# V-DETR/V-DETR

Hardware: AMD Instinct MI355X
Metric: scenes/sec (train fwd+bwd) 40k-pt ScanNet (higher is better)
Workload: dtype f32

## Files before the change

### v-detr_amd/csrc/attn_fwd_pipe.hip

```cpp
#include "attn_common.h"

namespace vdetr {

constexpr int kPT = 10;
constexpr int kPCells = kPT * kPT * kPT;
constexpr int kPipeThreads = 512;
constexpr int kPipeWaves = kPipeThreads / kWave;
constexpr int kPipePad = 20;
constexpr int kLdsPad = kRpeVerts * kPCells * 16;
constexpr int kLdsMl = kLdsPad + kPipeWaves * 16 * kPipePad * 4;
constexpr int kLdsXch = kLdsMl + kPipeWaves * 4 * 8 * 4;
constexpr int kLdsNext = kLdsXch + kPipeWaves * 8 * kWave * 4;
constexpr int kPipeLdsBytes = kLdsNext + 16;
constexpr int kPipeZeroCell = kPipeLdsBytes / 16;
constexpr int kPipeLdsBytesNearest = kPipeLdsBytes + 16;
static_assert(kPipeLdsBytes % 16 == 0 && kPipeLdsBytesNearest <= 160 * 1024, "the zero cell is a 16-byte slot inside the 160 KB LDS");

typedef float f32x2 __attribute__((ext_vector_type(2)));

struct PipeArgs {
  AttnParams P;
  unsigned* counter;
  int nitems, qtiles;
  const char* kv_img;
  int q_f32;
};

__device__ __forceinline__ AxisTap pipe_axis(float d, float log_scale, float pix_mul, float pix_add) {
  const float L = __log2f(__builtin_fmaf(fabsf(d), log_scale, 1.0f));
  const float pix = __builtin_fmaf(copysignf(L, d), pix_mul, pix_add);
  const float bf = __builtin_amdgcn_fmed3f(floorf(pix), 0.f, (float)(kPT - 2));
  const float t = pix - bf;
  AxisTap a;
  a.base = (int)bf;
  a.wa = sat01(1.f - fabsf(t));
  a.wb = sat01(1.f - fabsf(t - 1.f));
  return a;
}

struct PipeCorners {
  f32x4 c[8];
};
__device__ __forceinline__ void pipe_read8(const f32x4* t, PipeCorners& C) {
  C.c[0] = t[0]; C.c[1] = t[1]; C.c[2] = t[kPT]; C.c[3] = t[kPT + 1];
  C.c[4] = t[kPT * kPT]; C.c[5] = t[kPT * kPT + 1]; C.c[6] = t[kPT * kPT + kPT]; C.c[7] = t[kPT * kPT + kPT + 1];
}
__device__ __forceinline__ void pipe_fma8(const PipeCorners& C, float axa, float axb, float w00, float w01, float w10, float w11,
                                          f32x2& s01, f32x2& s23) {
  const float w[8] = {axa * w00, axb * w00, axa * w01, axb * w01, axa * w10, axb * w10, axa * w11, axb * w11};
#pragma unroll
  for (int k = 0; k < 8; ++k) {
    s01 = __builtin_elementwise_fma(f32x2{C.c[k][0], C.c[k][1]}, f32x2{w[k], w[k]}, s01);
    s23 = __builtin_elementwise_fma(f32x2{C.c[k][2], C.c[k][3]}, f32x2{w[k], w[k]}, s23);
  }
}

struct PipeQuery {
  float x0, x1, y0, y1, z0, z1;
  float rc, rs;
};

template <bool ROT, bool NEAREST>
__device__ __forceinline__ void pipe_bias_box(const AttnParams& P, const f32x4* tab, const PipeQuery& Q, float kx, float ky, float kz,
                                              f32x2& s01, f32x2& s23) {
  float dx[2], dy[2], dz[2];
  if (ROT) {
    float ax0 = Q.x0 - kx, ay0 = Q.y0 - ky;
    rpe_rotate(ax0, ay0, Q.rc, Q.rs);
    dx[0] = ax0; dx[1] = ax0 + Q.x1;
    dy[0] = ay0; dy[1] = ay0 + Q.y1;
    dz[0] = Q.z0 - kz; dz[1] = dz[0] + Q.z1;
  } else {
    dx[0] = Q.x0 - kx; dx[1] = Q.x1 - kx;
    dy[0] = Q.y0 - ky; dy[1] = Q.y1 - ky;
    dz[0] = Q.z0 - kz; dz[1] = Q.z1 - kz;
  }
  if constexpr (NEAREST) {
    int cx[2], cy[2], cz[2];
#pragma unroll
    for (int a = 0; a < 2; ++a) {
      cx[a] = rpe_axis_nearest(dx[a], P.log_scale, P.pix_mul, P.pix_add, kPT, 1);
      cy[a] = rpe_axis_nearest(dy[a], P.log_scale, P.pix_mul, P.pix_add, kPT, kPT);
      cz[a] = rpe_axis_nearest(dz[a], P.log_scale, P.pix_mul, P.pix_add, kPT, kPT * kPT);
    }
    f32x4 cv[kRpeVerts];
#pragma unroll
    for (int i = 0; i < kRpeVerts; ++i)
      cv[i] = tab[min(i * kPCells + cz[rpe_box_zi(i)] + cy[rpe_box_yi(i)] + cx[rpe_box_xi(i)], kPipeZeroCell)];
#pragma unroll
    for (int i = 0; i < kRpeVerts; ++i) {
      s01 += f32x2{cv[i][0], cv[i][1]};
      s23 += f32x2{cv[i][2], cv[i][3]};
    }
    return;
  }
  const AxisTap ax[2] = {pipe_axis(dx[0], P.log_scale, P.pix_mul, P.pix_add), pipe_axis(dx[1], P.log_scale, P.pix_mul, P.pix_add)};
  const AxisTap ay[2] = {pipe_axis(dy[0], P.log_scale, P.pix_mul, P.pix_add), pipe_axis(dy[1], P.log_scale, P.pix_mul, P.pix_add)};
  const AxisTap az[2] = {pipe_axis(dz[0], P.log_scale, P.pix_mul, P.pix_add), pipe_axis(dz[1], P.log_scale, P.pix_mul, P.pix_add)};
  float w00[2][2], w01[2][2], w10[2][2], w11[2][2];
  int zy[2][2];
#pragma unroll
  for (int zi = 0; zi < 2; ++zi)
#pragma unroll
    for (int yi = 0; yi < 2; ++yi) {
      w00[zi][yi] = az[zi].wa * ay[yi].wa; w01[zi][yi] = az[zi].wa * ay[yi].wb;
      w10[zi][yi] = az[zi].wb * ay[yi].wa; w11[zi][yi] = az[zi].wb * ay[yi].wb;
      zy[zi][yi] = __mul24(__mul24(az[zi].base, kPT) + ay[yi].base, kPT);
    }
  PipeCorners cur, nxt;
  pipe_read8(tab + zy[rpe_box_zi(0)][rpe_box_yi(0)] + ax[rpe_box_xi(0)].base, cur);
#pragma unroll
  for (int i = 0; i < kRpeVerts; ++i) {
    const int xi = rpe_box_xi(i), yi = rpe_box_yi(i), zi = rpe_box_zi(i);
    if (i + 1 < kRpeVerts)
      pipe_read8(tab + (i + 1) * kPCells + zy[rpe_box_zi(i + 1)][rpe_box_yi(i + 1)] + ax[rpe_box_xi(i + 1)].base, nxt);
    __builtin_amdgcn_sched_barrier(0);
    pipe_fma8(cur, ax[xi].wa, ax[xi].wb, w00[zi][yi], w01[zi][yi], w10[zi][yi], w11[zi][yi], s01, s23);
    if (i + 1 < kRpeVerts) cur = nxt;
  }
}

template <bool NEAREST>
__device__ __forceinline__ void pipe_bias_general(const AttnParams& P, const f32x4* tab, const float* __restrict__ vp, bool rot, float rc,
                                                  float rs, float kx, float ky, float kz, f32x2& s01, f32x2& s23) {
#pragma unroll 1
  for (int i = 0; i < kRpeVerts; ++i) {
    float dx = vp[i * 3] - kx, dy = vp[i * 3 + 1] - ky;
    const float dz = vp[i * 3 + 2] - kz;
    if (rot) rpe_rotate(dx, dy, rc, rs);
    if constexpr (NEAREST) {
      const int cell = rpe_axis_nearest(dx, P.log_scale, P.pix_mul, P.pix_add, kPT, 1) +
                       rpe_axis_nearest(dy, P.log_scale, P.pix_mul, P.pix_add, kPT, kPT) +
                       rpe_axis_nearest(dz, P.log_scale, P.pix_mul, P.pix_add, kPT, kPT * kPT);
      const f32x4 cv = tab[min(i * kPCells + cell, kPipeZeroCell)];
      s01 += f32x2{cv[0], cv[1]};
      s23 += f32x2{cv[2], cv[3]};
      continue;
    }
    const AxisTap ax = pipe_axis(dx, P.log_scale, P.pix_mul, P.pix_add), ay = pipe_axis(dy, P.log_scale, P.pix_mul, P.pix_add),
                  az = pipe_axis(dz, P.log_scale, P.pix_mul, P.pix_add);
    PipeCorners C;
    pipe_read8(tab + i * kPCells + (az.base * kPT + ay.base) * kPT + ax.base, C);
    pipe_fma8(C, ax.wa, ax.wb, az.wa * ay.wa, az.wa * ay.wb, az.wb * ay.wa, az.wb * ay.wb, s01, s23);
  }
}

__device__ __forceinline__ float pipe_give_back(float v, bool swapped, bool odd_row) {
  const auto r = __builtin_amdgcn_permlane16_swap(__float_as_uint(v), __float_as_uint(v), false, false);
  const float other = __uint_as_float(odd_row ? r[0] : r[1]);
  return swapped ? other : v;
}

enum { kPipeBox = 0, kPipeBoxRot = 1, kPipeGeneral = 2 };

typedef __bf16 bf16x8 __attribute__((ext_vector_type(8)));
typedef __bf16 bf16x4 __attribute__((ext_vector_type(4)));
typedef short short4v __attribute__((ext_vector_type(4)));

constexpr int pipe_k_pieces(int split) { return split == 1 ? 2 : 6; }
constexpr int pipe_v_pieces(int split) { return split == 1 ? 2 : 4; }
constexpr int pipe_tile_bytes(int split) { return (pipe_k_pieces(split) + pipe_v_pieces(split)) * kWave * 16; }

template <int SPLIT>
struct PipeTileT {
  f32x4 kb[SPLIT ? 1 : 4], vb[SPLIT ? 1 : 4];
  bf16x8 k8[SPLIT ? pipe_k_pieces(SPLIT) : 1];
  f32x4 v8[SPLIT ? pipe_v_pieces(SPLIT) : 1];
  float kx, ky, kz;
};

__device__ __forceinline__ void split3(float x, __bf16& h, __bf16& m, __bf16& l) {
  h = (__bf16)x;
  const float r1 = x - (float)h;
  m = (__bf16)r1;
  l = (__bf16)(r1 - (float)m);
}

struct PipeLane {
  const float* kp;
  const float* vp;
  const float* xp;
  float* sp;
  const char* img;
};

template <int SPLIT>
__device__ __forceinline__ void pipe_fetch_k(const AttnParams& P, const PipeLane& A, int tile, int nK, int c, PipeTileT<SPLIT>& t) {
  if constexpr (SPLIT) {
    const char* src = A.img + (size_t)tile * pipe_tile_bytes(SPLIT);
#pragma unroll
    for (int j = 0; j < pipe_k_pieces(SPLIT); ++j) t.k8[j] = *reinterpret_cast<const bf16x8*>(src + j * kWave * 16);
  } else {
    const int kc = min((tile << 4) + c, nK - 1) - c;
    const f32x4* kp = reinterpret_cast<const f32x4*>(A.kp + kc * P.k_stride);
#pragma unroll
    for (int s4 = 0; s4 < 4; ++s4) t.kb[s4] = kp[s4];
  }
}
template <int SPLIT>
__device__ __forceinline__ void pipe_fetch_x(const PipeLane& A, int tile, int nK, int c, PipeTileT<SPLIT>& t) {
  const int kc = min((tile << 4) + c, nK - 1) - c;
  const float* xp = A.xp + kc * 3;
  t.kx = xp[0]; t.ky = xp[1]; t.kz = xp[2];
}
template <int SPLIT>
__device__ __forceinline__ void pipe_fetch_v(const AttnParams& P, const PipeLane& A, int tile, int nK, int g, PipeTileT<SPLIT>& t) {
  if constexpr (SPLIT) {
    const char* src = A.img + (size_t)tile * pipe_tile_bytes(SPLIT) + pipe_k_pieces(SPLIT) * kWave * 16;
#pragma unroll
    for (int j = 0; j < pipe_v_pieces(SPLIT); ++j) t.v8[j] = *reinterpret_cast<const f32x4*>(src + j * kWave * 16);
  } else {
#pragma unroll
    for (int s = 0; s < 4; ++s) {
      const int kk = min((tile << 4) + 4 * g + s, nK - 1) - 4 * g;
      t.vb[s] = *reinterpret_cast<const f32x4*>(A.vp + kk * P.v_stride);
    }
  }
}

template <int SPLIT>
struct PipeQT {
  float qa[SPLIT ? 1 : 16];
  bf16x8 q8[SPLIT ? pipe_k_pieces(SPLIT) : 1];
};

template <int MODE, bool TAIL, int SPLIT, bool NEAREST>
__device__ __forceinline__ void pipe_tile(const AttnParams& P, const f32x4* tab, float* ppad, const PipeLane& A, const PipeQuery& Q,
                                          const float* __restrict__ role_vp, const PipeQT<SPLIT>& QA, PipeTileT<SPLIT>& ops, int tile, int next, int b,
                                          int qrow, int g, int c, bool swapped, f32x4 (&o)[4], float (&m)[4], float (&l)[4]) {
  const int nK = P.nK;
  const int key = (tile << 4) + c;
  const bool kvalid = !TAIL || key < nK;
  f32x4 acc = {0.f, 0.f, 0.f, 0.f};
  if constexpr (SPLIT == 1) {
    acc = __builtin_amdgcn_mfma_f32_16x16x32_bf16(QA.q8[0], ops.k8[0], acc, 0, 0, 0);
    acc = __builtin_amdgcn_mfma_f32_16x16x32_bf16(QA.q8[1], ops.k8[1], acc, 0, 0, 0);
    acc *= P.scale;
  } else if constexpr (SPLIT) {
    constexpr int kTerms[6][2] = {{2, 0}, {0, 2}, {1, 1}, {1, 0}, {0, 1}, {0, 0}};
#pragma unroll
    for (int t = 0; t < 6; ++t)
#pragma unroll
      for (int mm = 0; mm < 2; ++mm)
        acc = __builtin_amdgcn_mfma_f32_16x16x32_bf16(QA.q8[2 * kTerms[t][0] + mm], ops.k8[2 * kTerms[t][1] + mm], acc, 0, 0, 0);
  } else {
#pragma unroll
    for (int s = 0; s < 16; ++s) acc = __builtin_amdgcn_mfma_f32_16x16x4f32(QA.qa[s], ops.kb[s >> 2][s & 3], acc, 0, 0, 0);
  }
  if constexpr (!SPLIT) pipe_fetch_k<SPLIT>(P, A, next, nK, c, ops);
  const float kx = ops.kx, ky = ops.ky, kz = ops.kz;
  pipe_fetch_x<SPLIT>(A, next, nK, c, ops);
  f32x2 s01 = {0.f, 0.f}, s23 = {0.f, 0.f};
  if (MODE == kPipeGeneral) pipe_bias_general<NEAREST>(P, tab, role_vp, P.cos_sin != nullptr, Q.rc, Q.rs, kx, ky, kz, s01, s23);
  else pipe_bias_box<MODE == kPipeBoxRot, NEAREST>(P, tab, Q, kx, ky, kz, s01, s23);
  if constexpr (SPLIT) {
    __builtin_amdgcn_sched_barrier(0);
    pipe_fetch_k<SPLIT>(P, A, next, nK, c, ops);
    __builtin_amdgcn_sched_barrier(0);
  }
  const bool odd = g & 1;
  float sc[4];
  sc[0] = acc[0] + pipe_give_back(s01[0], swapped, odd);
  sc[1] = acc[1] + pipe_give_back(s01[1], swapped, odd);
  sc[2] = acc[2] + pipe_give_back(s23[0], swapped, odd);
  sc[3] = acc[3] + pipe_give_back(s23[1], swapped, odd);
  if (TAIL && !kvalid) {
#pragma unroll
    for (int r = 0; r < 4; ++r) sc[r] = kNegBig;
  }
  if (A.sp && kvalid && qrow < P.nQ) {
    float* sp = A.sp + (tile << 4);
#pragma unroll
    for (int r = 0; r < 4; ++r) {
      __builtin_nontemporal_store(sc[r], sp + r * nK);
    }
  }
  float p[4];
#pragma unroll
  for (int r = 0; r < 4; ++r) {
    const float tmax = row_allmax_f32_fx(sc[r]);
    const float mn = fmaxf(m[r], tmax);
    const float alpha = __expf(m[r] - mn);
    const float e = kvalid ? __expf(sc[r] - mn) : 0.f;
    l[r] = l[r] * alpha + row_allsum_f32_fx(e);
    m[r] = mn;
    p[r] = e;
#pragma unroll
    for (int t = 0; t < 4; ++t) o[t][r] *= alpha;
  }
  if (P.drop_thresh) {
    const uint4 rnd = attn_rand4(P, b, qrow, key, 0);
    p[0] = rnd.x >= P.drop_thresh ? p[0] * P.drop_scale : 0.f;
    p[1] = rnd.y >= P.drop_thresh ? p[1] * P.drop_scale : 0.f;
    p[2] = rnd.z >= P.drop_thresh ? p[2] * P.drop_scale : 0.f;
    p[3] = rnd.w >= P.drop_thresh ? p[3] * P.drop_scale : 0.f;
  }
#pragma unroll
  for (int r = 0; r < 4; ++r) ppad[(4 * g + r) * kPipePad + c] = p[r];
  __builtin_amdgcn_wave_barrier();
  const f32x4 pa = *reinterpret_cast<const f32x4*>(ppad + c * kPipePad + 4 * g);
  __builtin_amdgcn_wave_barrier();
  if constexpr (SPLIT == 1) {
    const bf16x4 pb = {(__bf16)pa[0], (__bf16)pa[1], (__bf16)pa[2], (__bf16)pa[3]};
    const short4v ab = __builtin_bit_cast(short4v, pb);
    typedef short short8v __attribute__((ext_vector_type(8)));
#pragma unroll
    for (int t = 0; t < 4; ++t) {
      const short8v vv = __builtin_bit_cast(short8v, ops.v8[t >> 1]);
      const short4v vt = (t & 1) ? short4v{vv[4], vv[5], vv[6], vv[7]} : short4v{vv[0], vv[1], vv[2], vv[3]};
      o[t] = __builtin_amdgcn_mfma_f32_16x16x16bf16_1k(ab, vt, o[t], 0, 0, 0);
    }
  } else if constexpr (SPLIT) {
    bf16x4 ph, pl;
#pragma unroll
    for (int e = 0; e < 4; ++e) {
      const __bf16 h = (__bf16)pa[e];
      ph[e] = h;
      pl[e] = (__bf16)(pa[e] - (float)h);
    }
    const short4v ah = __builtin_bit_cast(short4v, ph), al = __builtin_bit_cast(short4v, pl);
#pragma unroll
    for (int t = 0; t < 4; ++t) {
      typedef short short8v __attribute__((ext_vector_type(8)));
      const short8v vv = __builtin_bit_cast(short8v, ops.v8[t]);
      const short4v vh = {vv[0], vv[1], vv[2], vv[3]}, vl = {vv[4], vv[5], vv[6], vv[7]};
      o[t] = __builtin_amdgcn_mfma_f32_16x16x16bf16_1k(al, vh, o[t], 0, 0, 0);
      o[t] = __builtin_amdgcn_mfma_f32_16x16x16bf16_1k(ah, vl, o[t], 0, 0, 0);
      o[t] = __builtin_amdgcn_mfma_f32_16x16x16bf16_1k(ah, vh, o[t], 0, 0, 0);
    }
  } else {
#pragma unroll
    for (int t = 0; t < 4; ++t)
#pragma unroll
      for (int s = 0; s < 4; ++s) o[t] = __builtin_amdgcn_mfma_f32_16x16x4f32(pa[s], ops.vb[s][t], o[t], 0, 0, 0);
  }
  pipe_fetch_v<SPLIT>(P, A, next, nK, g, ops);
}

template <int MODE, int SPLIT, bool NEAREST>
__device__ __forceinline__ void pipe_tiles(const AttnParams& P, const f32x4* tab, float* ppad, const PipeLane& A, const PipeQuery& Q,
                                           const float* __restrict__ role_vp, const PipeQT<SPLIT>& qa, PipeTileT<SPLIT>& ops, int tile_begin,
                                           int tile_end, int w, int b, int qrow, int g, int c, bool swapped, f32x4 (&o)[4],
                                           float (&m)[4], float (&l)[4]) {
  const int nK = P.nK;
  const int full_end = min(tile_end, nK >> 4);
  int tile = tile_begin + w;
  for (; tile < full_end; tile += kPipeWaves) {
    const int next = tile + kPipeWaves < tile_end ? tile + kPipeWaves : tile;
    pipe_tile<MODE, false, SPLIT, NEAREST>(P, tab, ppad, A, Q, role_vp, qa, ops, tile, next, b, qrow, g, c, swapped, o, m, l);
  }
  if (tile < tile_end)
    pipe_tile<MODE, true, SPLIT, NEAREST>(P, tab, ppad, A, Q, role_vp, qa, ops, tile, tile, b, qrow, g, c, swapped, o, m, l);
}

template <bool ROT, int SPLIT, bool NEAREST = false>
__global__ __launch_bounds__(kPipeThreads) void attn_fwd_rpe_pipe_kernel(PipeArgs K) {
  extern __shared__ __attribute__((aligned(16))) float smem[];
  AttnParams& P = K.P;
  attn_load_rng(P);
  const int tid = threadIdx.x, lane = tid & 63;
  const int w = __builtin_amdgcn_readfirstlane(tid >> 6);
  const int g = lane >> 4, c = lane & 15;
  const bool swapped = c >= 4 && c < 12;
  const int gq = swapped ? (g ^ 1) : g;
  const int nQ = P.nQ, nK = P.nK, H = 4;
  const f32x4* tab = reinterpret_cast<const f32x4*>(smem);
  float* ppad = smem + kLdsPad / 4 + w * (16 * kPipePad);
  float* mlbuf = smem + kLdsMl / 4;
  float* xch = smem + kLdsXch / 4;
  volatile int* nextbuf = reinterpret_cast<volatile int*>(smem + kLdsNext / 4);

  const int last_draw = K.nitems + (int)gridDim.x - 1;
  if (tid == 0) {
    const int first = (int)atomicAdd(K.counter, 1u);
    nextbuf[0] = first;
    if (first == last_draw) atomicExch(K.counter, 0u);
  }
  if ((int)blockIdx.x + 8 >= (int)gridDim.x) {
    __syncthreads();
    if (nextbuf[0] >= K.nitems) return;
  }
  rpe_stage_table(P, reinterpret_cast<f32x4*>(smem), tid, kPipeThreads);
  if (NEAREST && tid == 0) reinterpret_cast<f32x4*>(smem)[kPipeZeroCell] = f32x4{0.f, 0.f, 0.f, 0.f};
  __syncthreads();
  int item = nextbuf[0];
  int parity = 0;
  const int ntiles = (nK + 15) >> 4;
  const int qstride = H * kDh;

  while (item < K.nitems) {
    int drawn = 0;
    if (tid == 0) drawn = (int)atomicAdd(K.counter, 1u);
    const int split = item % P.ksplit;
    const int qt = (item / P.ksplit) % K.qtiles;
    const int b = item / (P.ksplit * K.qtiles);
    const int q0 = qt * 4;
    const int tile_begin = split * P.tiles_per_split;
    const int tile_end = min(ntiles, tile_begin + P.tiles_per_split);
    const int qrow = q0 + g;
    const int q_role = min(q0 + gq, nQ - 1);
    PipeQT<SPLIT> qa;
    {
      const int qi = min(q0 + (c >> 2), nQ - 1);
      const float* qrowp = P.q + ((size_t)b * nQ + qi) * qstride + (c & 3) * kDh;
      if constexpr (SPLIT == 1) {
        if (K.q_f32) {
#pragma unroll
          for (int mm = 0; mm < 2; ++mm) {
            const f32x4* src = reinterpret_cast<const f32x4*>(qrowp + 32 * mm + 8 * g);
            const f32x4 v0 = src[0], v1 = src[1];
#pragma unroll
            for (int e = 0; e < 8; ++e) qa.q8[mm][e] = (__bf16)(e < 4 ? v0[e] : v1[e - 4]);
          }
        } else {
          const __bf16* qb = reinterpret_cast<const __bf16*>(P.q) + ((size_t)b * nQ + qi) * qstride + (c & 3) * kDh;
          qa.q8[0] = *reinterpret_cast<const bf16x8*>(qb + 8 * g);
          qa.q8[1] = *reinterpret_cast<const bf16x8*>(qb + 32 + 8 * g);
        }
      } else if constexpr (SPLIT) {
#pragma unroll
        for (int mm = 0; mm < 2; ++mm) {
          const f32x4* src = reinterpret_cast<const f32x4*>(qrowp + 32 * mm + 8 * g);
          const f32x4 v0 = src[0], v1 = src[1];
#pragma unroll
          for (int e = 0; e < 8; ++e) {
            __bf16 h, md, lo;
            split3((e < 4 ? v0[e] : v1[e - 4]) * P.scale, h, md, lo);
            qa.q8[mm][e] = h; qa.q8[2 + mm][e] = md; qa.q8[4 + mm][e] = lo;
          }
        }
      } else {
        const f32x4* src = reinterpret_cast<const f32x4*>(qrowp + 16 * g);
#pragma unroll
        for (int s4 = 0; s4 < 4; ++s4) {
          const f32x4 v = src[s4];
#pragma unroll
          for (int e = 0; e < 4; ++e) qa.qa[s4 * 4 + e] = v[e] * P.scale;
        }
      }
    }
    const float* role_vp = P.vertices + ((size_t)b * nQ + q_role) * 24;
    PipeQuery Q;
    Q.rc = 1.f; Q.rs = 0.f;
    bool box;
    {
      float vx[8], vy[8], vz[8];
#pragma unroll
      for (int i = 0; i < 8; ++i) { vx[i] = role_vp[i * 3]; vy[i] = role_vp[i * 3 + 1]; vz[i] = role_vp[i * 3 + 2]; }
      if (ROT) {
        Q.rc = P.cos_sin[((size_t)b * nQ + q_role) * 2];
        Q.rs = P.cos_sin[((size_t)b * nQ + q_role) * 2 + 1];
        float ex, ey, ez;
        box = __all(rpe_box_pattern_rot(vx, vy, vz, Q.rc, Q.rs, ex, ey, ez));
        Q.x0 = vx[0]; Q.y0 = vy[0]; Q.z0 = vz[0];
        Q.x1 = ex; Q.y1 = ey; Q.z1 = ez;
      } else {
        box = __all(rpe_box_pattern(vx, vy, vz));
        Q.x0 = vx[0]; Q.x1 = vx[2]; Q.y0 = vy[0]; Q.y1 = vy[1]; Q.z0 = vz[0]; Q.z1 = vz[4];
      }
    }
    PipeLane A;
    A.kp = P.k + ((size_t)b * nK + c) * P.k_stride + 16 * g;
    A.vp = P.v + ((size_t)b * nK + 4 * g) * P.v_stride + 4 * c;
    A.xp = P.xyz + ((size_t)b * nK + c) * 3;
    A.sp = P.scores ? P.scores + (((size_t)b * nQ + min(qrow, nQ - 1)) * H) * nK + c : nullptr;
    A.img = SPLIT ? K.kv_img + ((size_t)b * ntiles) * pipe_tile_bytes(SPLIT) + lane * 16 : nullptr;

    f32x4 o[4];
#pragma unroll
    for (int t = 0; t < 4; ++t) o[t] = f32x4{0.f, 0.f, 0.f, 0.f};
    float m[4] = {kNegBig, kNegBig, kNegBig, kNegBig}, l[4] = {0.f, 0.f, 0.f, 0.f};
    PipeTileT<SPLIT> ops;
    {
      const int t0 = min(tile_begin + w, ntiles - 1);
      pipe_fetch_k<SPLIT>(P, A, t0, nK, c, ops);
      pipe_fetch_x<SPLIT>(A, t0, nK, c, ops);
      pipe_fetch_v<SPLIT>(P, A, t0, nK, g, ops);
    }
    if (box)
      pipe_tiles<ROT ? kPipeBoxRot : kPipeBox, SPLIT, NEAREST>(P, tab, ppad, A, Q, role_vp, qa, ops, tile_begin, tile_end, w, b, qrow, g, c, swapped, o, m, l);
    else
      pipe_tiles<kPipeGeneral, SPLIT, NEAREST>(P, tab, ppad, A, Q, role_vp, qa, ops, tile_begin, tile_end, w, b, qrow, g, c, swapped, o, m, l);

    if (tid == 0) {
      nextbuf[parity ^ 1] = drawn;
      if (drawn == last_draw) atomicExch(K.counter, 0u);
    }
    __syncthreads();
    if (c == 0) {
      float* mine = mlbuf + (w * 4 + g) * 8;
      *reinterpret_cast<f32x4*>(mine) = f32x4{m[0], m[1], m[2], m[3]};
      *reinterpret_cast<f32x4*>(mine + 4) = f32x4{l[0], l[1], l[2], l[3]};
    }
    const int own_t = w >> 1, own_hi = w & 1;
#pragma unroll
    for (int half = 0; half < 2; ++half) {
      if (half) __syncthreads();
#pragma unroll
      for (int t = 0; t < 4; ++t)
#pragma unroll
        for (int hi = 0; hi < 2; ++hi) xch[(w * 8 + t * 2 + hi) * kWave + lane] = o[t][2 * hi + half];
      __syncthreads();
      const int r = 2 * own_hi + half;
      float M = kNegBig;
      float mw[kPipeWaves], lw[kPipeWaves];
#pragma unroll
      for (int ww = 0; ww < kPipeWaves; ++ww) {
        mw[ww] = mlbuf[(ww * 4 + g) * 8 + r];
        lw[ww] = mlbuf[(ww * 4 + g) * 8 + 4 + r];
        M = fmaxf(M, mw[ww]);
      }
      float L = 0.f, val = 0.f;
#pragma unroll
      for (int ww = 0; ww < kPipeWaves; ++ww) {
        const float f = __expf(mw[ww] - M);
        L += lw[ww] * f;
        val += xch[(ww * 8 + own_t * 2 + own_hi) * kWave + lane] * f;
      }
      if (qrow < nQ) {
        const float inv = L > 0.f ? 1.f / L : 0.f;
        const float lse = L > 0.f ? M + __logf(L) : kNegBig;
        const int d = 4 * c + own_t;
        const size_t row = ((size_t)b * nQ + qrow) * H + r;
        if (P.ksplit == 1) {
          P.out[row * kDh + d] = val * inv;
          if (own_t == 0 && c == 0) P.lse[row] = lse;
        } else {
          const size_t rows = (size_t)P.B * nQ * H;
          P.part_o[((size_t)split * rows + row) * kDh + d] = val * inv;
          if (own_t == 0 && c == 0) P.part_lse[(size_t)split * rows + row] = lse;
        }
      }
    }
    parity ^= 1;
    item = nextbuf[parity];
  }
}


template <int SPLIT, bool SRC_F32 = (SPLIT != 1)>
__global__ __launch_bounds__(kWave) void attn_fwd_pack_kv_kernel(const void* __restrict__ kin, const void* __restrict__ vin, int nK, int k_stride,
                                                                 int v_stride, char* __restrict__ img, long layer_stride, int nB) {
  const int lane = threadIdx.x, g = lane >> 4, c = lane & 15;
  const int tile = blockIdx.x, b = blockIdx.y, ntiles = gridDim.x;
  {
    const size_t esz = SRC_F32 ? 4 : 2;
    kin = reinterpret_cast<const char*>(kin) + (size_t)blockIdx.z * layer_stride * esz;
    vin = reinterpret_cast<const char*>(vin) + (size_t)blockIdx.z * layer_stride * esz;
    img += (size_t)blockIdx.z * nB * ntiles * pipe_tile_bytes(SPLIT);
  }
  char* dst = img + ((size_t)b * ntiles + tile) * pipe_tile_bytes(SPLIT) + lane * 16;
  const int key = tile * 16 + c;
  constexpr int kK = pipe_k_pieces(SPLIT);
  if constexpr (SPLIT == 1 && SRC_F32) {
    const float* k = reinterpret_cast<const float*>(kin);
    const float* v = reinterpret_cast<const float*>(vin);
    const float* kr = k + ((size_t)b * nK + min(key, nK - 1)) * k_stride;
#pragma unroll
    for (int mm = 0; mm < 2; ++mm) {
      const f32x4 v0 = *reinterpret_cast<const f32x4*>(kr + 32 * mm + 8 * g), v1 = *reinterpret_cast<const f32x4*>(kr + 32 * mm + 8 * g + 4);
      bf16x8 h;
#pragma unroll
      for (int e = 0; e < 8; ++e) h[e] = (__bf16)(key < nK ? (e < 4 ? v0[e] : v1[e - 4]) : 0.f);
      *reinterpret_cast<bf16x8*>(dst + mm * kWave * 16) = h;
    }
#pragma unroll
    for (int tp = 0; tp < 2; ++tp) {
      bf16x8 both;
#pragma unroll
      for (int e = 0; e < 4; ++e) {
        const int kk = tile * 16 + 4 * g + e;
        const float* vr = v + ((size_t)b * nK + min(kk, nK - 1)) * v_stride + 4 * c + 2 * tp;
        both[e] = (__bf16)(kk < nK ? vr[0] : 0.f);
        both[4 + e] = (__bf16)(kk < nK ? vr[1] : 0.f);
      }
      *reinterpret_cast<bf16x8*>(dst + (kK + tp) * kWave * 16) = both;
    }
  } else if constexpr (SPLIT == 1) {
    const __bf16* k = reinterpret_cast<const __bf16*>(kin);
    const __bf16* v = reinterpret_cast<const __bf16*>(vin);
    const __bf16* kr = k + ((size_t)b * nK + min(key, nK - 1)) * k_stride;
    const bf16x8 zero8 = {0, 0, 0, 0, 0, 0, 0, 0};
#pragma unroll
    for (int mm = 0; mm < 2; ++mm)
      *reinterpret_cast<bf16x8*>(dst + mm * kWave * 16) = key < nK ? *reinterpret_cast<const bf16x8*>(kr + 32 * mm + 8 * g) : zero8;
#pragma unroll
    for (int tp = 0; tp < 2; ++tp) {
      bf16x8 both;
#pragma unroll
      for (int e = 0; e < 4; ++e) {
        const int kk = tile * 16 + 4 * g + e;
        const __bf16* vr = v + ((size_t)b * nK + min(kk, nK - 1)) * v_stride + 4 * c + 2 * tp;
        both[e] = kk < nK ? vr[0] : (__bf16)0.f;
        both[4 + e] = kk < nK ? vr[1] : (__bf16)0.f;
      }
      *reinterpret_cast<bf16x8*>(dst + (kK + tp) * kWave * 16) = both;
    }
  } else {
    const float* k = reinterpret_cast<const float*>(kin);
    const float* v = reinterpret_cast<const float*>(vin);
    const float* kr = k + ((size_t)b * nK + min(key, nK - 1)) * k_stride;
#pragma unroll
    for (int mm = 0; mm < 2; ++mm) {
      const f32x4 v0 = *reinterpret_cast<const f32x4*>(kr + 32 * mm + 8 * g), v1 = *reinterpret_cast<const f32x4*>(kr + 32 * mm + 8 * g + 4);
      bf16x8 h, md, lo;
#pragma unroll
      for (int e = 0; e < 8; ++e) {
        __bf16 a0, a1, a2;
        split3(key < nK ? (e < 4 ? v0[e] : v1[e - 4]) : 0.f, a0, a1, a2);
        h[e] = a0; md[e] = a1; lo[e] = a2;
      }
      *reinterpret_cast<bf16x8*>(dst + (0 + mm) * kWave * 16) = h;
      *reinterpret_cast<bf16x8*>(dst + (2 + mm) * kWave * 16) = md;
      *reinterpret_cast<bf16x8*>(dst + (4 + mm) * kWave * 16) = lo;
    }
#pragma unroll
    for (int t = 0; t < 4; ++t) {
      bf16x4 h, lo;
#pragma unroll
      for (int e = 0; e < 4; ++e) {
        const int kk = tile * 16 + 4 * g + e;
        const float x = kk < nK ? v[((size_t)b * nK + kk) * v_stride + 4 * c + t] : 0.f;
        const __bf16 hh = (__bf16)x;
        h[e] = hh;
        lo[e] = (__bf16)(x - (float)hh);
      }
      bf16x8 both = {h[0], h[1], h[2], h[3], lo[0], lo[1], lo[2], lo[3]};
      *reinterpret_cast<bf16x8*>(dst + (kK + t) * kWave * 16) = both;
    }
  }
}

}

using namespace vdetr;

namespace vdetr {
size_t attn_fwd_pipe_img_bytes(int B, int nK, int split) { return (size_t)B * ((nK + 15) / 16) * (split == 1 ? pipe_tile_bytes(1) : pipe_tile_bytes(3)); }

int attn_fwd_pack_launch(const void* k, const void* v, int B, int nK, int k_stride, int v_stride, int nlayers, long layer_stride, char* img,
                         int split, bool src_f32, hipStream_t st) {
  const dim3 pg((nK + 15) / 16, B, nlayers);
  if (split == 1 && src_f32) hipLaunchKernelGGL((attn_fwd_pack_kv_kernel<1, true>), pg, dim3(kWave), 0, st, k, v, nK, k_stride, v_stride, img, layer_stride, B);
  else if (split == 1) hipLaunchKernelGGL((attn_fwd_pack_kv_kernel<1, false>), pg, dim3(kWave), 0, st, k, v, nK, k_stride, v_stride, img, layer_stride, B);
  else hipLaunchKernelGGL(attn_fwd_pack_kv_kernel<3>, pg, dim3(kWave), 0, st, k, v, nK, k_stride, v_stride, img, layer_stride, B);
  return check_launch("attn_fwd_pack_kv");
}

int attn_fwd_pipe_launch(const AttnParams& P, unsigned* counter, int workgroups, char* kv_img, int split, bool packed, bool src_f32, hipStream_t st) {
  PipeArgs K;
  K.P = P;
  K.counter = counter;
  K.qtiles = (P.nQ + 3) / 4;
  K.nitems = P.B * K.qtiles * P.ksplit;
  K.kv_img = kv_img;
  K.q_f32 = src_f32 ? 1 : 0;
  const int grid = workgroups < K.nitems ? workgroups : K.nitems;
  if (split && !packed) {
    if (int e = attn_fwd_pack_launch(P.k, P.v, P.B, P.nK, P.k_stride, P.v_stride, 1, 0, kv_img, split, src_f32, st)) return e;
  }
#define VDETR_PIPE_LAUNCH(ROT, SPLIT)                                                                                       \
  do {                                                                                                                      \
    if (P.rpe_nearest) {                                                                                                    \
      if (int e = set_lds(attn_fwd_rpe_pipe_kernel<ROT, SPLIT, true>, kPipeLdsBytesNearest, "attn_fwd")) return e;         \
      hipLaunchKernelGGL((attn_fwd_rpe_pipe_kernel<ROT, SPLIT, true>), dim3(grid), dim3(kPipeThreads), kPipeLdsBytesNearest, st, K); \
    } else {                                                                                                                \
      if (int e = set_lds(attn_fwd_rpe_pipe_kernel<ROT, SPLIT>, kPipeLdsBytes, "attn_fwd")) return e;                      \
      hipLaunchKernelGGL((attn_fwd_rpe_pipe_kernel<ROT, SPLIT>), dim3(grid), dim3(kPipeThreads), kPipeLdsBytes, st, K);    \
    }                                                                                                                       \
  } while (0)
  if (P.cos_sin) {
    if (split == 1) VDETR_PIPE_LAUNCH(true, 1); else if (split) VDETR_PIPE_LAUNCH(true, 3); else VDETR_PIPE_LAUNCH(true, 0);
  } else {
    if (split == 1) VDETR_PIPE_LAUNCH(false, 1); else if (split) VDETR_PIPE_LAUNCH(false, 3); else VDETR_PIPE_LAUNCH(false, 0);
  }
#undef VDETR_PIPE_LAUNCH
  return check_launch("attn_fwd_pipe");
}
}
```

Before: 156.6.

## Prefetch next work item's K/V, query rows and vertices across persistent-loop boundary

The persistent attention forward kernel now draws two work items up front. It prefetches the next item's first K/V/xyz tile inside the last tile iteration and stages that item's query rows, box vertices and cos/sin into LDS during the epilogue, which hides the refill latency between items. The RPE table load is issued into registers before the first synchronisation, item decoding uses precomputed magic-number division, and an optional compile-time timeline instrumentation is added. This adds about 4.5 KB of LDS and extra register pressure, and it makes the counter handling more intricate.

```diff
diff --git a/v-detr_amd/csrc/attn_fwd_pipe.hip b/v-detr_amd/csrc/attn_fwd_pipe.hip
--- a/v-detr_amd/csrc/attn_fwd_pipe.hip
+++ b/v-detr_amd/csrc/attn_fwd_pipe.hip
@@ -11,10 +11,15 @@
 constexpr int kLdsMl = kLdsPad + kPipeWaves * 16 * kPipePad * 4;
 constexpr int kLdsXch = kLdsMl + kPipeWaves * 4 * 8 * 4;
 constexpr int kLdsNext = kLdsXch + kPipeWaves * 8 * kWave * 4;
-constexpr int kPipeLdsBytes = kLdsNext + 16;
+constexpr int kLdsStage = kLdsNext + 16;
+constexpr int kPipeStageFloats = 4 * 256 + 4 * 24 + 4 * 2;
+constexpr int kPipeLdsBytes = kLdsStage + kPipeStageFloats * 4;
 constexpr int kPipeZeroCell = kPipeLdsBytes / 16;
 constexpr int kPipeLdsBytesNearest = kPipeLdsBytes + 16;
 static_assert(kPipeLdsBytes % 16 == 0 && kPipeLdsBytesNearest <= 160 * 1024, "the zero cell is a 16-byte slot inside the 160 KB LDS");
+static_assert(kLdsPad == kRpeVerts * kPCells * 16 && kLdsMl - kLdsPad == kPipeWaves * 16 * kPipePad * 4 && kLdsXch - kLdsMl == 1024 &&
+                  kLdsNext - kLdsXch == 16384 && kLdsStage - kLdsNext == 16 && kLdsStage % 16 == 0 && kPipeLdsBytes - kLdsStage == 4512,
+              "LDS map: table, P pads, m / l, exchange, item indices, staged item; the staged q rows are read as 16-byte pieces");
 
 typedef float f32x2 __attribute__((ext_vector_type(2)));
 
@@ -22,9 +27,30 @@
   AttnParams P;
   unsigned* counter;
   int nitems, qtiles;
+  unsigned ks_mul, ks_sh, qt_mul, qt_sh;
   const char* kv_img;
   int q_f32;
+#ifdef VDETR_PIPE_TIMELINE
+  unsigned long long* tl;
+#endif
 };
+
+#ifdef VDETR_PIPE_TIMELINE
+constexpr int kPipeTlItems = 60;
+constexpr int kPipeTlWords = 4 + 4 * kPipeTlItems;
+static unsigned long long* g_pipe_timeline = nullptr;
+#define PIPE_TL(word)                                                                                                   \
+  do {                                                                                                                  \
+    if (K.tl && tid == 0 && (word) < kPipeTlWords) K.tl[(size_t)blockIdx.x * kPipeTlWords + (word)] = wall_clock64();   \
+  } while (0)
+#define PIPE_TL_SET(word, value)                                                                                        \
+  do {                                                                                                                  \
+    if (K.tl && tid == 0) K.tl[(size_t)blockIdx.x * kPipeTlWords + (word)] = (value);                                   \
+  } while (0)
+#else
+#define PIPE_TL(word) do { } while (0)
+#define PIPE_TL_SET(word, value) do { } while (0)
+#endif
 
 __device__ __forceinline__ AxisTap pipe_axis(float d, float log_scale, float pix_mul, float pix_add) {
   const float L = __log2f(__builtin_fmaf(fabsf(d), log_scale, 1.0f));
@@ -176,44 +202,48 @@
   l = (__bf16)(r1 - (float)m);
 }
 
-struct PipeLane {
-  const float* kp;
-  const float* vp;
-  const float* xp;
-  float* sp;
+struct PipeSrc {
+  const float* k;
+  const float* v;
+  const float* xyz;
   const char* img;
 };
+__device__ __forceinline__ PipeSrc pipe_pick(bool first, const PipeSrc& a, const PipeSrc& b) {
+  PipeSrc r;
+  r.k = first ? a.k : b.k; r.v = first ? a.v : b.v; r.xyz = first ? a.xyz : b.xyz; r.img = first ? a.img : b.img;
+  return r;
+}
 
 template <int SPLIT>
-__device__ __forceinline__ void pipe_fetch_k(const AttnParams& P, const PipeLane& A, int tile, int nK, int c, PipeTileT<SPLIT>& t) {
+__device__ __forceinline__ void pipe_fetch_k(const AttnParams& P, const PipeSrc& A, int tile, int nK, int g, int c, PipeTileT<SPLIT>& t) {
   if constexpr (SPLIT) {
-    const char* src = A.img + (size_t)tile * pipe_tile_bytes(SPLIT);
+    const char* src = A.img + (size_t)tile * pipe_tile_bytes(SPLIT) + (g * 16 + c) * 16;
 #pragma unroll
     for (int j = 0; j < pipe_k_pieces(SPLIT); ++j) t.k8[j] = *reinterpret_cast<const bf16x8*>(src + j * kWave * 16);
   } else {
-    const int kc = min((tile << 4) + c, nK - 1) - c;
-    const f32x4* kp = reinterpret_cast<const f32x4*>(A.kp + kc * P.k_stride);
+    const int kc = min((tile << 4) + c, nK - 1);
+    const f32x4* kp = reinterpret_cast<const f32x4*>(A.k + kc * P.k_stride + 16 * g);
 #pragma unroll
     for (int s4 = 0; s4 < 4; ++s4) t.kb[s4] = kp[s4];
   }
 }
 template <int SPLIT>
-__device__ __forceinline__ void pipe_fetch_x(const PipeLane& A, int tile, int nK, int c, PipeTileT<SPLIT>& t) {
-  const int kc = min((tile << 4) + c, nK - 1) - c;
-  const float* xp = A.xp + kc * 3;
+__device__ __forceinline__ void pipe_fetch_x(const PipeSrc& A, int tile, int nK, int c, PipeTileT<SPLIT>& t) {
+  const int kc = min((tile << 4) + c, nK - 1);
+  const float* xp = A.xyz + kc * 3;
   t.kx = xp[0]; t.ky = xp[1]; t.kz = xp[2];
 }
 template <int SPLIT>
-__device__ __forceinline__ void pipe_fetch_v(const AttnParams& P, const PipeLane& A, int tile, int nK, int g, PipeTileT<SPLIT>& t) {
+__device__ __forceinline__ void pipe_fetch_v(const AttnParams& P, const PipeSrc& A, int tile, int nK, int g, int c, PipeTileT<SPLIT>& t) {
   if constexpr (SPLIT) {
-    const char* src = A.img + (size_t)tile * pipe_tile_bytes(SPLIT) + pipe_k_pieces(SPLIT) * kWave * 16;
+    const char* src = A.img + (size_t)tile * pipe_tile_bytes(SPLIT) + (pipe_k_pieces(SPLIT) * kWave + g * 16 + c) * 16;
 #pragma unroll
     for (int j = 0; j < pipe_v_pieces(SPLIT); ++j) t.v8[j] = *reinterpret_cast<const f32x4*>(src + j * kWave * 16);
   } else {
 #pragma unroll
     for (int s = 0; s < 4; ++s) {
-      const int kk = min((tile << 4) + 4 * g + s, nK - 1) - 4 * g;
-      t.vb[s] = *reinterpret_cast<const f32x4*>(A.vp + kk * P.v_stride);
+      const int kk = min((tile << 4) + 4 * g + s, nK - 1);
+      t.vb[s] = *reinterpret_cast<const f32x4*>(A.v + kk * P.v_stride + 4 * c);
     }
   }
 }
@@ -225,7 +255,7 @@
 };
 
 template <int MODE, bool TAIL, int SPLIT, bool NEAREST>
-__device__ __forceinline__ void pipe_tile(const AttnParams& P, const f32x4* tab, float* ppad, const PipeLane& A, const PipeQuery& Q,
+__device__ __forceinline__ void pipe_tile(const AttnParams& P, const f32x4* tab, float* ppad, float* sp_row, const PipeSrc& A, const PipeQuery& Q,
                                           const float* __restrict__ role_vp, const PipeQT<SPLIT>& QA, PipeTileT<SPLIT>& ops, int tile, int next, int b,
                                           int qrow, int g, int c, bool swapped, f32x4 (&o)[4], float (&m)[4], float (&l)[4]) {
   const int nK = P.nK;
@@ -247,7 +277,7 @@
 #pragma unroll
     for (int s = 0; s < 16; ++s) acc = __builtin_amdgcn_mfma_f32_16x16x4f32(QA.qa[s], ops.kb[s >> 2][s & 3], acc, 0, 0, 0);
   }
-  if constexpr (!SPLIT) pipe_fetch_k<SPLIT>(P, A, next, nK, c, ops);
+  if constexpr (!SPLIT) pipe_fetch_k<SPLIT>(P, A, next, nK, g, c, ops);
   const float kx = ops.kx, ky = ops.ky, kz = ops.kz;
   pipe_fetch_x<SPLIT>(A, next, nK, c, ops);
   f32x2 s01 = {0.f, 0.f}, s23 = {0.f, 0.f};
@@ -255,7 +285,7 @@
   else pipe_bias_box<MODE == kPipeBoxRot, NEAREST>(P, tab, Q, kx, ky, kz, s01, s23);
   if constexpr (SPLIT) {
     __builtin_amdgcn_sched_barrier(0);
-    pipe_fetch_k<SPLIT>(P, A, next, nK, c, ops);
+    pipe_fetch_k<SPLIT>(P, A, next, nK, g, c, ops);
     __builtin_amdgcn_sched_barrier(0);
   }
   const bool odd = g & 1;
@@ -268,8 +298,8 @@
 #pragma unroll
     for (int r = 0; r < 4; ++r) sc[r] = kNegBig;
   }
-  if (A.sp && kvalid && qrow < P.nQ) {
-    float* sp = A.sp + (tile << 4);
+  if (sp_row && kvalid && qrow < P.nQ) {
+    float* sp = sp_row + (tile << 4);
 #pragma unroll
     for (int r = 0; r < 4; ++r) {
       __builtin_nontemporal_store(sc[r], sp + r * nK);
@@ -334,23 +364,53 @@
 #pragma unroll
       for (int s = 0; s < 4; ++s) o[t] = __builtin_amdgcn_mfma_f32_16x16x4f32(pa[s], ops.vb[s][t], o[t], 0, 0, 0);
   }
-  pipe_fetch_v<SPLIT>(P, A, next, nK, g, ops);
+  pipe_fetch_v<SPLIT>(P, A, next, nK, g, c, ops);
 }
 
 template <int MODE, int SPLIT, bool NEAREST>
-__device__ __forceinline__ void pipe_tiles(const AttnParams& P, const f32x4* tab, float* ppad, const PipeLane& A, const PipeQuery& Q,
-                                           const float* __restrict__ role_vp, const PipeQT<SPLIT>& qa, PipeTileT<SPLIT>& ops, int tile_begin,
-                                           int tile_end, int w, int b, int qrow, int g, int c, bool swapped, f32x4 (&o)[4],
-                                           float (&m)[4], float (&l)[4]) {
+__device__ __forceinline__ void pipe_tiles(const AttnParams& P, const f32x4* tab, float* ppad, float* sp_row, const PipeSrc& A, const PipeSrc& An, int tn,
+                                           const PipeQuery& Q, const float* __restrict__ role_vp, const PipeQT<SPLIT>& qa, PipeTileT<SPLIT>& ops,
+                                           int tile_begin, int tile_end, int w, int b, int qrow, int g, int c, bool swapped, f32x4 (&o)[4],
+                                           float (&m)[4], float (&l)[4], unsigned long long* tl_first) {
   const int nK = P.nK;
   const int full_end = min(tile_end, nK >> 4);
   int tile = tile_begin + w;
   for (; tile < full_end; tile += kPipeWaves) {
-    const int next = tile + kPipeWaves < tile_end ? tile + kPipeWaves : tile;
-    pipe_tile<MODE, false, SPLIT, NEAREST>(P, tab, ppad, A, Q, role_vp, qa, ops, tile, next, b, qrow, g, c, swapped, o, m, l);
+    const bool more = tile + kPipeWaves < tile_end;
+    const int next = more ? tile + kPipeWaves : tn;
+    const PipeSrc F = pipe_pick(more, A, An);
+    pipe_tile<MODE, false, SPLIT, NEAREST>(P, tab, ppad, sp_row, F, Q, role_vp, qa, ops, tile, next, b, qrow, g, c, swapped, o, m, l);
+    if (tl_first) { *tl_first = wall_clock64(); tl_first = nullptr; }
   }
   if (tile < tile_end)
-    pipe_tile<MODE, true, SPLIT, NEAREST>(P, tab, ppad, A, Q, role_vp, qa, ops, tile, tile, b, qrow, g, c, swapped, o, m, l);
+    pipe_tile<MODE, true, SPLIT, NEAREST>(P, tab, ppad, sp_row, An, Q, role_vp, qa, ops, tile, tn, b, qrow, g, c, swapped, o, m, l);
+  if (tl_first) *tl_first = wall_clock64();
+}
+
+struct PipeItem {
+  int split, q0, b, tile_begin, tile_end;
+};
+__device__ __forceinline__ unsigned pipe_div(unsigned n, unsigned mul, unsigned sh) { return (unsigned)(((unsigned long long)n * mul) >> sh); }
+__device__ __forceinline__ PipeItem pipe_item(const PipeArgs& K, int item, int ntiles) {
+  const unsigned iq = pipe_div((unsigned)item, K.ks_mul, K.ks_sh);
+  const unsigned b = pipe_div(iq, K.qt_mul, K.qt_sh);
+  PipeItem I;
+  I.split = item - (int)iq * K.P.ksplit;
+  I.q0 = ((int)iq - (int)b * K.qtiles) * 4;
+  I.b = (int)b;
+  I.tile_begin = I.split * K.P.tiles_per_split;
+  I.tile_end = min(ntiles, I.tile_begin + K.P.tiles_per_split);
+  return I;
+}
+template <int SPLIT>
+__device__ __forceinline__ PipeSrc pipe_src(const PipeArgs& K, int b, int ntiles) {
+  const AttnParams& P = K.P;
+  PipeSrc A;
+  A.k = P.k + (size_t)b * P.nK * P.k_stride;
+  A.v = P.v + (size_t)b * P.nK * P.v_stride;
+  A.xyz = P.xyz + (size_t)b * P.nK * 3;
+  A.img = SPLIT ? K.kv_img + ((size_t)b * ntiles) * pipe_tile_bytes(SPLIT) : nullptr;
+  return A;
 }
 
 template <bool ROT, int SPLIT, bool NEAREST = false>
@@ -368,41 +428,116 @@
   float* ppad = smem + kLdsPad / 4 + w * (16 * kPipePad);
   float* mlbuf = smem + kLdsMl / 4;
   float* xch = smem + kLdsXch / 4;
-  volatile int* nextbuf = reinterpret_cast<volatile int*>(smem + kLdsNext / 4);
-
-  const int last_draw = K.nitems + (int)gridDim.x - 1;
-  if (tid == 0) {
-    const int first = (int)atomicAdd(K.counter, 1u);
-    nextbuf[0] = first;
-    if (first == last_draw) atomicExch(K.counter, 0u);
-  }
-  if ((int)blockIdx.x + 8 >= (int)gridDim.x) {
-    __syncthreads();
-    if (nextbuf[0] >= K.nitems) return;
-  }
-  rpe_stage_table(P, reinterpret_cast<f32x4*>(smem), tid, kPipeThreads);
-  if (NEAREST && tid == 0) reinterpret_cast<f32x4*>(smem)[kPipeZeroCell] = f32x4{0.f, 0.f, 0.f, 0.f};
-  __syncthreads();
-  int item = nextbuf[0];
-  int parity = 0;
+  int* nextbuf = reinterpret_cast<int*>(smem + kLdsNext / 4);
+  float* stq = smem + kLdsStage / 4;
+  float* stv = stq + 4 * 256;
+  float* stc = stv + 4 * 24;
   const int ntiles = (nK + 15) >> 4;
   const int qstride = H * kDh;
-
-  while (item < K.nitems) {
-    int drawn = 0;
-    if (tid == 0) drawn = (int)atomicAdd(K.counter, 1u);
-    const int split = item % P.ksplit;
-    const int qt = (item / P.ksplit) % K.qtiles;
-    const int b = item / (P.ksplit * K.qtiles);
-    const int q0 = qt * 4;
-    const int tile_begin = split * P.tiles_per_split;
-    const int tile_end = min(ntiles, tile_begin + P.tiles_per_split);
+  const bool q_bf16 = SPLIT == 1 && !K.q_f32;
+
+  const int last_draw = K.nitems + (int)gridDim.x - 1;
+  PIPE_TL(1);
+  unsigned counter_off = 0;
+  asm volatile("" : "+v"(counter_off));
+  unsigned* const counter = K.counter + counter_off;
+  int first = 0;
+  if (tid == 0) first = (int)atomicAdd(counter, 1u);
+  const bool late = (int)blockIdx.x + 8 >= (int)gridDim.x;
+  constexpr int kCells = kRpeVerts * kPCells, kTabBatch = (kCells + kPipeThreads - 1) / kPipeThreads;
+  f32x4 tv[kTabBatch];
+  auto table_request = [&]() {
+    const f32x4* src = reinterpret_cast<const f32x4*>(P.table);
+#pragma unroll
+    for (int u = 0; u < kTabBatch; ++u) {
+      const int cell = tid + u * kPipeThreads;
+      tv[u] = src[min(cell, kCells - 1)];
+    }
+  };
+  if (!late) table_request();
+  if (tid == 0) {
+    if (first == last_draw) atomicExch(K.counter, 0u);
+    int second = K.nitems;
+    if (first < K.nitems) {
+      second = (int)atomicAdd(K.counter, 1u);
+      if (second == last_draw) atomicExch(K.counter, 0u);
+    }
+    nextbuf[0] = first;
+    nextbuf[1] = second;
+  }
+  __syncthreads();
+  int item = __builtin_amdgcn_readfirstlane(nextbuf[0]);
+  int nxt = __builtin_amdgcn_readfirstlane(nextbuf[1]);
+  if (item >= K.nitems) return;
+  if (late) table_request();
+
+  f32x4 st_q;
+  float st_f;
+  auto stage_request = [&](const PipeItem& I) {
+    const int j = w & 3;
+    const int qi = min(I.q0 + (q_bf16 ? (lane >> 5) + 2 * (j & 1) : j), nQ - 1);
+    const size_t qoff = ((size_t)I.b * nQ + qi) * qstride;
+    const char* qsrc = q_bf16 ? reinterpret_cast<const char*>(reinterpret_cast<const __bf16*>(P.q) + qoff) + (lane & 31) * 16
+                              : reinterpret_cast<const char*>(P.q + qoff) + lane * 16;
+    st_q = *reinterpret_cast<const f32x4*>(qsrc);
+    const int idx = tid & 127;
+    const int e = idx < 96 ? idx : 0, vj = e / 24;
+    const float* fsrc = P.vertices + ((size_t)I.b * nQ + min(I.q0 + vj, nQ - 1)) * 24 + (e - 24 * vj);
+    if (ROT) {
+      const float* csrc = P.cos_sin + ((size_t)I.b * nQ + min(I.q0 + ((idx >> 1) & 3), nQ - 1)) * 2 + (idx & 1);
+      fsrc = idx >= 96 && idx < 104 ? csrc : fsrc;
+    }
+    st_f = *fsrc;
+  };
+  auto stage_store = [&]() {
+    if (w < (q_bf16 ? 2 : 4)) {
+      reinterpret_cast<f32x4*>(stq)[tid] = st_q;
+    } else if (w >= 4 && w < 6) {
+      const int idx = tid & 127;
+      if (idx < 96) stv[idx] = st_f;
+      else if (ROT && idx < 104) stc[idx - 96] = st_f;
+    }
+  };
+
+  PipeItem I = pipe_item(K, item, ntiles);
+  PipeTileT<SPLIT> ops;
+  {
+    stage_request(I);
+    const PipeSrc A0 = pipe_src<SPLIT>(K, I.b, ntiles);
+    const int t0 = min(I.tile_begin + w, ntiles - 1);
+    pipe_fetch_k<SPLIT>(P, A0, t0, nK, g, c, ops);
+    pipe_fetch_x<SPLIT>(A0, t0, nK, c, ops);
+    pipe_fetch_v<SPLIT>(P, A0, t0, nK, g, c, ops);
+  }
+  {
+    f32x4* dst = reinterpret_cast<f32x4*>(smem);
+#pragma unroll
+    for (int u = 0; u < kTabBatch; ++u) {
+      const int cell = tid + u * kPipeThreads;
+      if (cell < kCells) dst[cell] = tv[u];
+    }
+  }
+  if (NEAREST && tid == 0) reinterpret_cast<f32x4*>(smem)[kPipeZeroCell] = f32x4{0.f, 0.f, 0.f, 0.f};
+  stage_store();
+  __syncthreads();
+  PIPE_TL(2);
+  int parity = 0;
+#ifdef VDETR_PIPE_TIMELINE
+  int tl_n = 0;
+#endif
+
+  while (true) {
+    const bool has_next = nxt < K.nitems;
+    const int split = I.split, b = I.b, q0 = I.q0;
+    const int tile_begin = I.tile_begin, tile_end = I.tile_end;
+    const PipeItem In = has_next ? pipe_item(K, nxt, ntiles) : I;
+    const PipeSrc A = pipe_src<SPLIT>(K, b, ntiles), An = pipe_src<SPLIT>(K, In.b, ntiles);
+    const int tn = min(In.tile_begin + w, ntiles - 1);
     const int qrow = q0 + g;
     const int q_role = min(q0 + gq, nQ - 1);
     PipeQT<SPLIT> qa;
     {
-      const int qi = min(q0 + (c >> 2), nQ - 1);
-      const float* qrowp = P.q + ((size_t)b * nQ + qi) * qstride + (c & 3) * kDh;
+      const float* qrowp = stq + (c >> 2) * qstride + (c & 3) * kDh;
       if constexpr (SPLIT == 1) {
         if (K.q_f32) {
 #pragma unroll
@@ -413,7 +548,7 @@
             for (int e = 0; e < 8; ++e) qa.q8[mm][e] = (__bf16)(e < 4 ? v0[e] : v1[e - 4]);
           }
         } else {
-          const __bf16* qb = reinterpret_cast<const __bf16*>(P.q) + ((size_t)b * nQ + qi) * qstride + (c & 3) * kDh;
+          const __bf16* qb = reinterpret_cast<const __bf16*>(stq) + (c >> 2) * qstride + (c & 3) * kDh;
           qa.q8[0] = *reinterpret_cast<const bf16x8*>(qb + 8 * g);
           qa.q8[1] = *reinterpret_cast<const bf16x8*>(qb + 32 + 8 * g);
         }
@@ -445,11 +580,12 @@
     bool box;
     {
       float vx[8], vy[8], vz[8];
-#pragma unroll
-      for (int i = 0; i < 8; ++i) { vx[i] = role_vp[i * 3]; vy[i] = role_vp[i * 3 + 1]; vz[i] = role_vp[i * 3 + 2]; }
+      const float* sv = stv + gq * 24;
+#pragma unroll
+      for (int i = 0; i < 8; ++i) { vx[i] = sv[i * 3]; vy[i] = sv[i * 3 + 1]; vz[i] = sv[i * 3 + 2]; }
       if (ROT) {
-        Q.rc = P.cos_sin[((size_t)b * nQ + q_role) * 2];
-        Q.rs = P.cos_sin[((size_t)b * nQ + q_role) * 2 + 1];
+        Q.rc = stc[gq * 2];
+        Q.rs = stc[gq * 2 + 1];
         float ex, ey, ez;
         box = __all(rpe_box_pattern_rot(vx, vy, vz, Q.rc, Q.rs, ex, ey, ez));
         Q.x0 = vx[0]; Q.y0 = vy[0]; Q.z0 = vz[0];
@@ -459,33 +595,32 @@
         Q.x0 = vx[0]; Q.x1 = vx[2]; Q.y0 = vy[0]; Q.y1 = vy[1]; Q.z0 = vz[0]; Q.z1 = vz[4];
       }
     }
-    PipeLane A;
-    A.kp = P.k + ((size_t)b * nK + c) * P.k_stride + 16 * g;
-    A.vp = P.v + ((size_t)b * nK + 4 * g) * P.v_stride + 4 * c;
-    A.xp = P.xyz + ((size_t)b * nK + c) * 3;
-    A.sp = P.scores ? P.scores + (((size_t)b * nQ + min(qrow, nQ - 1)) * H) * nK + c : nullptr;
-    A.img = SPLIT ? K.kv_img + ((size_t)b * ntiles) * pipe_tile_bytes(SPLIT) + lane * 16 : nullptr;
+    float* sp_row = P.scores ? P.scores + (((size_t)b * nQ + min(qrow, nQ - 1)) * H) * nK + c : nullptr;
 
     f32x4 o[4];
 #pragma unroll
     for (int t = 0; t < 4; ++t) o[t] = f32x4{0.f, 0.f, 0.f, 0.f};
     float m[4] = {kNegBig, kNegBig, kNegBig, kNegBig}, l[4] = {0.f, 0.f, 0.f, 0.f};
-    PipeTileT<SPLIT> ops;
-    {
-      const int t0 = min(tile_begin + w, ntiles - 1);
-      pipe_fetch_k<SPLIT>(P, A, t0, nK, c, ops);
-      pipe_fetch_x<SPLIT>(A, t0, nK, c, ops);
-      pipe_fetch_v<SPLIT>(P, A, t0, nK, g, ops);
-    }
-    if (box)
-      pipe_tiles<ROT ? kPipeBoxRot : kPipeBox, SPLIT, NEAREST>(P, tab, ppad, A, Q, role_vp, qa, ops, tile_begin, tile_end, w, b, qrow, g, c, swapped, o, m, l);
-    else
-      pipe_tiles<kPipeGeneral, SPLIT, NEAREST>(P, tab, ppad, A, Q, role_vp, qa, ops, tile_begin, tile_end, w, b, qrow, g, c, swapped, o, m, l);
-
-    if (tid == 0) {
-      nextbuf[parity ^ 1] = drawn;
-      if (drawn == last_draw) atomicExch(K.counter, 0u);
-    }
+#ifdef VDETR_PIPE_TIMELINE
+    PIPE_TL(4 + 4 * tl_n);
+    unsigned long long* const tl_first = K.tl && tid == 0 && tl_n < kPipeTlItems ? K.tl + (size_t)blockIdx.x * kPipeTlWords + 5 + 4 * tl_n : nullptr;
+#else
+    unsigned long long* const tl_first = nullptr;
+#endif
+    if (tile_begin + w >= tile_end) {
+      pipe_fetch_k<SPLIT>(P, An, tn, nK, g, c, ops);
+      pipe_fetch_x<SPLIT>(An, tn, nK, c, ops);
+      pipe_fetch_v<SPLIT>(P, An, tn, nK, g, c, ops);
+    } else if (box) {
+      pipe_tiles<ROT ? kPipeBoxRot : kPipeBox, SPLIT, NEAREST>(P, tab, ppad, sp_row, A, An, tn, Q, role_vp, qa, ops, tile_begin, tile_end, w, b, qrow, g, c, swapped, o, m, l, tl_first);
+    } else {
+      pipe_tiles<kPipeGeneral, SPLIT, NEAREST>(P, tab, ppad, sp_row, A, An, tn, Q, role_vp, qa, ops, tile_begin, tile_end, w, b, qrow, g, c, swapped, o, m, l, tl_first);
+    }
+    PIPE_TL(6 + 4 * tl_n);
+    int drawn = K.nitems;
+    if (tid == 0 && has_next) drawn = (int)atomicAdd(counter, 1u);
+    stage_request(In);
+
     __syncthreads();
     if (c == 0) {
       float* mine = mlbuf + (w * 4 + g) * 8;
@@ -495,7 +630,14 @@
     const int own_t = w >> 1, own_hi = w & 1;
 #pragma unroll
     for (int half = 0; half < 2; ++half) {
-      if (half) __syncthreads();
+      if (half) {
+        __syncthreads();
+        stage_store();
+        if (tid == 0) {
+          nextbuf[2 + parity] = drawn;
+          if (drawn == last_draw) atomicExch(K.counter, 0u);
+        }
+      }
 #pragma unroll
       for (int t = 0; t < 4; ++t)
 #pragma unroll
@@ -532,8 +674,15 @@
         }
       }
     }
+#ifdef VDETR_PIPE_TIMELINE
+    PIPE_TL(7 + 4 * tl_n);
+    ++tl_n;
+    PIPE_TL_SET(0, (unsigned long long)tl_n);
+#endif
+    if (!has_next) break;
+    I = In;
+    nxt = __builtin_amdgcn_readfirstlane(nextbuf[2 + parity]);
     parity ^= 1;
-    item = nextbuf[parity];
   }
 }
 
@@ -635,6 +784,11 @@
 
 using namespace vdetr;
 
+#ifdef VDETR_PIPE_TIMELINE
+extern "C" int vdetr_attn_pipe_timeline_words(void) { return kPipeTlWords; }
+extern "C" void vdetr_attn_pipe_timeline_buffer(unsigned long long* buf) { g_pipe_timeline = buf; }
+#endif
+
 namespace vdetr {
 size_t attn_fwd_pipe_img_bytes(int B, int nK, int split) { return (size_t)B * ((nK + 15) / 16) * (split == 1 ? pipe_tile_bytes(1) : pipe_tile_bytes(3)); }
 
@@ -645,6 +799,13 @@
   else if (split == 1) hipLaunchKernelGGL((attn_fwd_pack_kv_kernel<1, false>), pg, dim3(kWave), 0, st, k, v, nK, k_stride, v_stride, img, layer_stride, B);
   else hipLaunchKernelGGL(attn_fwd_pack_kv_kernel<3>, pg, dim3(kWave), 0, st, k, v, nK, k_stride, v_stride, img, layer_stride, B);
   return check_launch("attn_fwd_pack_kv");
+}
+
+static void pipe_div_consts(unsigned d, unsigned& mul, unsigned& sh) {
+  unsigned s = 0;
+  while ((1ull << s) < d) ++s;
+  sh = 31 + s;
+  mul = (unsigned)(((1ull << sh) + d - 1) / d);
 }
 
 int attn_fwd_pipe_launch(const AttnParams& P, unsigned* counter, int workgroups, char* kv_img, int split, bool packed, bool src_f32, hipStream_t st) {
@@ -655,6 +816,15 @@
   K.nitems = P.B * K.qtiles * P.ksplit;
   K.kv_img = kv_img;
   K.q_f32 = src_f32 ? 1 : 0;
+  if ((long)P.B * K.qtiles * P.ksplit + workgroups >= (1L << 31)) {
+    set_error("attn_fwd: %ld items do not fit the persistent forward's 31-bit item index", (long)P.B * K.qtiles * P.ksplit);
+    return VDETR_ERR_ARG;
+  }
+  pipe_div_consts((unsigned)P.ksplit, K.ks_mul, K.ks_sh);
+  pipe_div_consts((unsigned)K.qtiles, K.qt_mul, K.qt_sh);
+#ifdef VDETR_PIPE_TIMELINE
+  K.tl = g_pipe_timeline;
+#endif
   const int grid = workgroups < K.nitems ? workgroups : K.nitems;
   if (split && !packed) {
     if (int e = attn_fwd_pack_launch(P.k, P.v, P.B, P.nK, P.k_stride, P.v_stride, 1, 0, kv_img, split, src_f32, st)) return e;
```

New measurement: 156.7, median of 2. No clear change (+0.1%).
